# RamSaw/PipelineDP

Hardware: AMD Instinct MI355X
Metric: records/sec DPEngine.aggregate COUNT+SUM at 1/2/4/8 MI355X; % HBM roofline (higher is better)
Workload: dtype f64; 1 GPU; configs[1]: 1e+09 records / 1e+07 privacy ids / 1e+06 Zipf(1.1) partitions per GPU, COUNT+SUM+PRIVACY_ID_COUNT, private partition selection; records_per_gpu=1000000000, privacy_ids_per_gpu=10000000, partitions=1000000, max_partitions_contributed=8, max_contributions_per_partition=2, noise=laplace, selection=truncated_geometric, parallelism=pid-sharded x1, privacy_id_range_supplied=True

## Files before the change

### pipelinedp_amd/csrc/dpg_team.h

```cpp
#pragma once

#include "dpg_partition.h"

namespace dpg {

constexpr int kTeamIPT = 16;
#ifndef DPG_TEAM_PF
#define DPG_TEAM_PF 1
#endif
#ifndef DPG_TEAM_PF_PC
#define DPG_TEAM_PF_PC 1
#endif
#ifndef DPG_TEAM_WB
#define DPG_TEAM_WB 4
#endif
#ifndef DPG_TEAM_PAIR
#define DPG_TEAM_PAIR 1
#endif
#ifndef DPG_TEAM_DESC_AHEAD
#define DPG_TEAM_DESC_AHEAD 0
#endif
#ifndef DPG_TEAM_SCAN1
#define DPG_TEAM_SCAN1 1
#endif
constexpr uint32_t kTeamF = 2048;
constexpr int kTeamSub = kScatThreads * kTeamIPT;
constexpr uint64_t kTeamTimeout = 50000000ull;
constexpr uint32_t kTeamArriveStride = 32;

struct TeamSync {
    uint32_t *tot;
    uint32_t *arrive;
    uint32_t *abort;
    uint32_t *err;
    uint32_t *paths = nullptr;
};

template <class R>
constexpr size_t team_lds() {
    return sizeof(R) * (kTeamSub + 1) + (size_t)kTeamF * 12 + 4 * 4 + 64;
}

__device__ __forceinline__ uint32_t ld_agent(const uint32_t *p) {
    return __hip_atomic_load(p, __ATOMIC_RELAXED, __HIP_MEMORY_SCOPE_AGENT);
}

struct NoOp {
    __device__ __forceinline__ void operator()() const {}
};
template <class F = NoOp>
__device__ __forceinline__ bool team_barrier(const TeamSync &ts, uint32_t team, uint32_t target,
                                             uint32_t *sh_ok, const F &between = F{}) {
    asm volatile("s_waitcnt vmcnt(0)" ::: "memory");
    __syncthreads();
    uint32_t *ctr = ts.arrive + team * kTeamArriveStride;
    uint32_t seen = 0;
    if (threadIdx.x == 0) {
        __hip_atomic_fetch_add(ctr, 1u, __ATOMIC_RELAXED, __HIP_MEMORY_SCOPE_AGENT);
        seen = ld_agent(ctr);
    }
    between();
    if (threadIdx.x == 0) {
        const uint64_t t0 = wall_clock64();
        uint32_t ok = 1;
        for (; seen < target; seen = ld_agent(ctr)) {
            if (ld_agent(ts.abort)) {
                ok = 0;
                break;
            }
            if (wall_clock64() - t0 > kTeamTimeout) {
                atomicOr(ts.abort, 1u);
                atomicOr(ts.err, 8u);
                ok = 0;
                break;
            }
            __builtin_amdgcn_s_sleep(2);
        }
        *sh_ok = ok;
    }
    __syncthreads();
    return *sh_ok != 0;
}

struct PieceDesc {
    uint32_t n;
    uint32_t pad0;
    int64_t ostart;
    int64_t base0;
    uint32_t ppre[8];
    uint32_t dl[8];
    uint32_t cend[8];
    uint32_t pad1[2];
};
static_assert(sizeof(PieceDesc) == 128, "PieceDesc is two 64-byte scalar loads");

struct PieceTab {
    const int64_t *rbase;
    const uint32_t *cum;
    const uint32_t *tot;
    const uint32_t *ptot;
    const int64_t *ostart;
    uint32_t F1;
    const PieceDesc *desc = nullptr;
};

typedef uint32_t u32x16 __attribute__((ext_vector_type(16)));
__device__ __forceinline__ void sload_desc(const PieceDesc *p, u32x16 &a, u32x16 &b) {
    p = uniform_ptr(p);
    asm volatile("s_load_dwordx16 %0, %2, 0x0\n\ts_load_dwordx16 %1, %2, 0x40\n\ts_waitcnt lgkmcnt(0)"
                 : "=s"(a), "=s"(b)
                 : "s"(p)
                 : "memory");
}
__device__ __forceinline__ void sload_desc_early(const PieceDesc *p, u32x16 &a, u32x16 &b) {
    typedef const u32x16 __attribute__((address_space(4))) * ConstVec;
    const ConstVec q = (ConstVec)(uintptr_t)uniform_ptr(p);
    a = q[0];
    b = q[1];
}

struct PieceSpan {
    uint32_t bnd, dl0, ce0, dl1, ce1, pair;
};
__host__ __device__ inline PieceSpan team_resolve(const uint32_t (&ppre)[8], const uint32_t (&dl)[8],
                                                  const uint32_t (&ce)[8], uint32_t b0, uint32_t lim) {
    const uint32_t i0 = b0, i1 = b0 + (lim > 2u ? lim : 2u) - 2u;
    PieceSpan r{ppre[0], dl[0], ce[0], dl[0], ce[0], 0u};
    const uint32_t n0 = ~i0, n1 = ~i1;
    uint32_t m0[8], m1[8];
#pragma unroll
    for (int p = 1; p < 8; ++p) {
        m0[p] = (uint32_t)((int32_t)(ppre[p] + n0) >> 31);
        m1[p] = (uint32_t)((int32_t)(ppre[p] + n1) >> 31);
#ifdef __HIP_DEVICE_COMPILE__
        asm("" : "+s"(m0[p]), "+s"(m1[p]));
#endif
        r.dl0 ^= (r.dl0 ^ dl[p]) & m0[p];
        r.ce0 ^= (r.ce0 ^ ce[p]) & m0[p];
        r.dl1 ^= (r.dl1 ^ dl[p]) & m1[p];
        r.ce1 ^= (r.ce1 ^ ce[p]) & m1[p];
        r.bnd ^= (r.bnd ^ ppre[p]) & m1[p];
    }
    uint32_t mid = 0;
#pragma unroll
    for (int p = 1; p < 7; ++p)
        mid |= ~m0[p] & m1[p + 1] & (uint32_t)((int32_t)(ppre[p] - ppre[p + 1]) >> 31);
    r.pair = ~mid & 1u;
    return r;
}

__device__ __forceinline__ uint32_t team_addr_lookup(const u32x16 &da, const u32x16 &db, uint32_t b0,
                                                     uint32_t lim, uint32_t (&boff)[kTeamIPT / 2]) {
    uint32_t ppre[8], dl[8], ce[8];
#pragma unroll
    for (int p = 0; p < 8; ++p) {
        ppre[p] = da[6 + p];
        dl[p] = p < 2 ? da[14 + p] : db[p - 2];
        ce[p] = db[6 + p];
    }
    uint32_t vm = 0;
#pragma unroll
    for (int mm = 0; mm < kTeamIPT / 2; ++mm) {
        const uint32_t o = mm * 2 * kScatThreads + 2 * threadIdx.x;
        const uint32_t i = b0 + min(o, lim - 2);
        uint32_t d = dl[0], c = ce[0];
#pragma unroll
        for (int p = 1; p < 8; ++p) {
            const bool in = i >= ppre[p];
            d = in ? dl[p] : d;
            c = in ? ce[p] : c;
        }
        boff[mm] = (i + d) * 8u;
        vm |= (i < c ? 1u : 0u) << (2 * mm);
        vm |= (i + 1 < c ? 1u : 0u) << (2 * mm + 1);
    }
    return vm;
}
__device__ __forceinline__ uint32_t team_addr_pair(const PieceSpan &sp, uint32_t b0, uint32_t lim,
                                                   uint32_t (&boff)[kTeamIPT / 2]) {
    uint32_t vm = 0;
#pragma unroll
    for (int mm = 0; mm < kTeamIPT / 2; ++mm) {
        const uint32_t o = mm * 2 * kScatThreads + 2 * threadIdx.x;
        const uint32_t i = b0 + min(o, lim - 2);
        const bool in = i >= sp.bnd;
        const uint32_t d = in ? sp.dl1 : sp.dl0, c = in ? sp.ce1 : sp.ce0;
        boff[mm] = (i + d) * 8u;
        vm |= (i < c ? 1u : 0u) << (2 * mm);
        vm |= (i + 1 < c ? 1u : 0u) << (2 * mm + 1);
    }
    return vm;
}
template <class R>
__device__ __forceinline__ void team_fetch(const R *a, int64_t base0, uint32_t (&boff)[kTeamIPT / 2],
                                           uint32_t &vm, R (&rec)[kTeamIPT]) {
    static_assert(sizeof(R) == 8 && kTeamIPT == 16, "piece-mode teams read 8-byte records");
    asm volatile(""
                 : "+v"(boff[0]), "+v"(boff[1]), "+v"(boff[2]), "+v"(boff[3]), "+v"(boff[4]),
                   "+v"(boff[5]), "+v"(boff[6]), "+v"(boff[7]), "+v"(vm));
    const char *bp = reinterpret_cast<const char *>(a + base0);
#pragma unroll
    for (int mm = 0; mm < kTeamIPT / 2; ++mm) {
        R x0, x1;
        const u64x2 w = *reinterpret_cast<const u64x2 *>(bp + boff[mm]);
        const uint64_t w0 = w.x, w1 = w.y;
        __builtin_memcpy(&x0, &w0, sizeof(R));
        __builtin_memcpy(&x1, &w1, sizeof(R));
        rec[2 * mm] = x0;
        rec[2 * mm + 1] = x1;
    }
}

template <class R, bool kPc = false, bool kMulti = false>
__global__ __launch_bounds__(kScatThreads) void k_part2_team(SrcAoS<R> src,
                                                             const int64_t *seg_start,
                                                             const uint32_t *seg_cnt, uint32_t S,
                                                             uint32_t F2, R *out, int64_t *base_out,
                                                             uint32_t *tot_out, TeamSync ts,
                                                             PieceTab pt = PieceTab{},
                                                             uint32_t sub_cap = kTeamSub) {
    constexpr int IPT = kTeamIPT;
    constexpr int SUB = kTeamSub;
    constexpr uint32_t F = kTeamF;
    constexpr int DPT = F / kScatThreads;
    using W = Words<R>;
    extern __shared__ __attribute__((aligned(16))) char smem[];
    W *stage = reinterpret_cast<W *>(smem);
    uint32_t *cnt = reinterpret_cast<uint32_t *>(smem + sizeof(R) * (SUB + 1));
    uint32_t *dstart = cnt + F;
    uint32_t *cur = dstart + F + 1;
    uint32_t *sh16 = cur + F;
    __shared__ uint32_t sh_ok;
    const uint32_t team = blockIdx.x & 7u;
    const uint32_t T = gridDim.x >> 3;
    const uint32_t m = blockIdx.x >> 3;
    const int tid = threadIdx.x;
    const int lane = tid & 63, wv = tid >> 6;
    for (uint32_t d = tid; d < F; d += kScatThreads) cnt[d] = 0;
    __syncthreads();
    auto elem = [tid](int j) -> uint32_t {
        return (uint32_t)((j >> 1) * 2 * kScatThreads + 2 * tid + (j & 1));
    };
    auto share = [&](uint32_t s, int64_t &st, uint32_t &n, uint32_t &b0, uint32_t &lim) {
        n = __builtin_amdgcn_readfirstlane(kPc ? pt.ptot[s] : seg_cnt[s]);
        const int64_t st0 = kPc ? pt.ostart[s] : seg_start[s];
        st = (int64_t)(((uint64_t)__builtin_amdgcn_readfirstlane((uint32_t)((uint64_t)st0 >> 32)) << 32) |
                       (uint32_t)__builtin_amdgcn_readfirstlane((uint32_t)st0));
        const uint32_t q = kPc ? (((n + T - 1) / T + 1) & ~1u) : (n + T - 1) / T;
        b0 = min(n, m * q);
        lim = min(n, b0 + q) - b0;
    };
    R rec[IPT];
    uint32_t vmask = ~0u;
    auto load = [&](int64_t base, uint32_t lim) {
        if (lim >= 2) {
#pragma unroll
            for (int mm = 0; mm < IPT / 2; ++mm) {
                const uint32_t o = mm * 2 * kScatThreads + 2 * tid;
                const uint32_t a = min(o, lim - 2);
                R x0, x1;
                src.fetch2(base + a, x0, x1);
                rec[2 * mm] = a == o ? x0 : x1;
                rec[2 * mm + 1] = x1;
            }
        } else {
#pragma unroll
            for (int j = 0; j < IPT; ++j) rec[j] = lim ? src.fetch(base) : R{};
        }
    };
    auto load_pieces = [&](uint32_t s, uint32_t b0, uint32_t lim) {
        uint32_t ppre[8], dl[8], pc[8];
        const int64_t rb0 = pt.rbase[s];
        const int64_t base0 = (int64_t)(((uint64_t)__builtin_amdgcn_readfirstlane((uint32_t)((uint64_t)rb0 >> 32)) << 32) |
                                        (uint32_t)__builtin_amdgcn_readfirstlane((uint32_t)rb0));
        uint32_t acc = 0;
#pragma unroll
        for (int p = 0; p < 8; ++p) {
            const uint32_t off = __builtin_amdgcn_readfirstlane(
                (uint32_t)(pt.rbase[(size_t)p * pt.F1 + s] - rb0));
            pc[p] = __builtin_amdgcn_readfirstlane(pt.cum[(size_t)p * pt.F1 + s]);
            ppre[p] = acc;
            dl[p] = off - acc;
            acc += (pc[p] + 1u) & ~1u;
        }
        const char *bp = reinterpret_cast<const char *>(src.a + base0);
        uint32_t vm = 0;
#pragma unroll
        for (int mm = 0; mm < IPT / 2; ++mm) {
            const uint32_t o = mm * 2 * kScatThreads + 2 * tid;
            const uint32_t i = b0 + min(o, lim - 2);
            uint32_t d = dl[0], c = pc[0] + ppre[0];
#pragma unroll
            for (int p = 1; p < 8; ++p) {
                const bool in = i >= ppre[p];
                d = in ? dl[p] : d;
                c = in ? pc[p] + ppre[p] : c;
            }
            R x0, x1;
            const uint32_t boff = (i + d) * (uint32_t)sizeof(R);
            static_assert(sizeof(R) == 8, "piece-mode teams read 8-byte records");
            const u64x2 w = *reinterpret_cast<const u64x2 *>(bp + boff);
            const uint64_t w0 = w.x, w1 = w.y;
            __builtin_memcpy(&x0, &w0, sizeof(R));
            __builtin_memcpy(&x1, &w1, sizeof(R));
            rec[2 * mm] = x0;
            rec[2 * mm + 1] = x1;
            vm |= (i < c ? 1u : 0u) << (2 * mm);
            vm |= (i + 1 < c ? 1u : 0u) << (2 * mm + 1);
        }
        vmask = vm;
    };
    auto load_pieces_desc = [&](const u32x16 &da, const u32x16 &db, uint32_t b0, uint32_t lim) {
        uint32_t boff[IPT / 2];
        uint32_t vm = team_addr_lookup(da, db, b0, lim, boff);
        team_fetch<R>(src.a, (int64_t)(((uint64_t)da[5] << 32) | da[4]), boff, vm, rec);
        vmask = vm;
    };
    auto load_span = [&](const PieceSpan &sp, int64_t base0, const PieceDesc *dp, uint32_t b0,
                         uint32_t lim) {
        uint32_t boff[IPT / 2];
        uint32_t vm;
        if (sp.pair) {
            vm = team_addr_pair(sp, b0, lim, boff);
        } else {
            u32x16 da, db;
            sload_desc(dp, da, db);
            vm = team_addr_lookup(da, db, b0, lim, boff);
        }
        team_fetch<R>(src.a, base0, boff, vm, rec);
        vmask = vm;
    };
    uint32_t k = 0;
    constexpr bool kPF = DPG_TEAM_PF && (!kPc || DPG_TEAM_PF_PC) && !kMulti;
    auto share_q = [&](uint32_t n) -> uint32_t {
        return kPc ? (((n + T - 1) / T + 1) & ~1u) : (n + T - 1) / T;
    };
    auto next_nonempty = [&](uint32_t s) -> uint32_t {
        for (; s < S; s += 8) {
            const uint32_t n = __builtin_amdgcn_readfirstlane(kPc ? pt.ptot[s] : seg_cnt[s]);
            if (n != 0 && share_q(n) <= sub_cap) break;
        }
        return s;
    };
    int64_t pf_st = 0;
    uint32_t pf_n = 0, pf_b0 = 0, pf_lim = 0;
    constexpr bool use_desc = kPc && kPF;
    constexpr bool kPair = use_desc && DPG_TEAM_PAIR;
    constexpr bool kAhead = use_desc && DPG_TEAM_DESC_AHEAD;
    PieceSpan pf_sp{};
    int64_t pf_base0 = 0;
    u32x16 pf_da = {}, pf_db = {};
    uint32_t n_pair = 0, n_lookup = 0;
    auto take_desc = [&](const u32x16 &da, const u32x16 &db) {
        pf_n = __builtin_amdgcn_readfirstlane(da[0]);
        pf_st = (int64_t)(((uint64_t)da[3] << 32) | da[2]);
        const uint32_t q = ((pf_n + T - 1) / T + 1) & ~1u;
        pf_b0 = min(pf_n, m * q);
        pf_lim = min(pf_n, pf_b0 + q) - pf_b0;
        if constexpr (kPair) {
            uint32_t ppre[8], dl[8], ce[8];
#pragma unroll
            for (int p = 0; p < 8; ++p) {
                ppre[p] = da[6 + p];
                dl[p] = p < 2 ? da[14 + p] : db[p - 2];
                ce[p] = db[6 + p];
            }
            pf_base0 = (int64_t)(((uint64_t)da[5] << 32) | da[4]);
            pf_sp = team_resolve(ppre, dl, ce, pf_b0, pf_lim);
            asm volatile(""
                         : "+s"(pf_sp.bnd), "+s"(pf_sp.dl0), "+s"(pf_sp.ce0), "+s"(pf_sp.dl1),
                           "+s"(pf_sp.ce1), "+s"(pf_sp.pair), "+s"(pf_b0), "+s"(pf_lim), "+s"(pf_base0));
        } else {
            pf_da = da;
            pf_db = db;
        }
    };
    auto issue_share = [&](uint32_t s) {
        if constexpr (kPair) {
            if (s < S) {
                n_pair += pf_sp.pair;
                n_lookup += 1u - pf_sp.pair;
            }
            load_span(pf_sp, pf_base0, pt.desc + min(s, S - 1), pf_b0, max(pf_lim, 2u));
        } else {
            load_pieces_desc(pf_da, pf_db, pf_b0, max(pf_lim, 2u));
        }
    };
    auto load_share = [&](uint32_t s) {
        if constexpr (kPc) {
            if constexpr (use_desc) {
                u32x16 da, db;
                sload_desc(pt.desc + min(s, S - 1), da, db);
                take_desc(da, db);
                issue_share(s);
                return;
            }
        }
        share(s, pf_st, pf_n, pf_b0, pf_lim);
        if constexpr (kPc) {
            vmask = 0;
            if (pf_lim > 0) load_pieces(s, pf_b0, pf_lim);
        } else {
            load(pf_st + pf_b0, pf_lim);
        }
    };
    uint32_t pf_s = S;
    if constexpr (kPF) {
        pf_s = next_nonempty(team);
        if (use_desc || pf_s < S) load_share(pf_s);
    }
    auto write_out = [&](int64_t st, uint32_t nv) {
        constexpr int WB = DPG_TEAM_WB;
        for (uint32_t k0 = 0; k0 < nv; k0 += WB * kScatThreads) {
            W x[WB];
            uint32_t dd[WB], kc[WB];
#pragma unroll
            for (int u = 0; u < WB; ++u) {
                kc[u] = min(k0 + u * kScatThreads + tid, nv - 1);
                x[u] = stage[kc[u]];
                dd[u] = src.digit(from_words<R>(x[u]));
            }
            uint32_t c1[WB], c2[WB];
#pragma unroll
            for (int u = 0; u < WB; ++u) {
                c1[u] = cur[dd[u]];
                c2[u] = dstart[dd[u]];
            }
#pragma unroll
            for (int u = 0; u < WB; ++u)
                *reinterpret_cast<W *>(&out[st + c1[u] + (kc[u] - c2[u])]) = x[u];
        }
    };
    for (uint32_t s = team; s < S; s += 8) {
        int64_t st;
        uint32_t n, b0, lim;
        if constexpr (kPF) {
            if (s == pf_s) {
                st = pf_st;
                n = pf_n;
                b0 = pf_b0;
                lim = pf_lim;
            } else {
                share(s, st, n, b0, lim);
            }
        } else {
            share(s, st, n, b0, lim);
        }
        if constexpr (kMulti) {
            if (n == 0 || share_q(n) <= sub_cap) continue;
        } else {
            if (n == 0) {
                if (m == 0)
                    for (uint32_t d = tid; d < F2; d += kScatThreads) {
                        base_out[(size_t)s * F2 + d] = st;
                        tot_out[(size_t)s * F2 + d] = 0;
                    }
                continue;
            }
            if (share_q(n) > sub_cap) continue;
        }
        auto team_starts = [&](const uint32_t *tt) {
            const uint32_t d0 = DPT * tid;
            uint32_t c[DPT], x = 0;
#pragma unroll
            for (int u = 0; u < DPT; ++u) {
                c[u] = ld_agent(&tt[d0 + u]);
                x += c[u];
            }
            uint32_t wt;
            uint32_t e = wave_excl_scan(x, wt);
            if (lane == 63) sh16[wv] = wt;
            __syncthreads();
#if DPG_TEAM_SCAN1
            uint32_t all;
            e += block_prefix16(sh16, all);
#else
#pragma unroll
            for (int w = 0; w < kScatThreads / 64; ++w)
                if (w < wv) e += sh16[w];
#endif
            uint32_t *tz = ts.tot + ((size_t)team * 3 + (k + 1) % 3) * F;
#pragma unroll
            for (int u = 0; u < DPT; ++u) {
                cur[d0 + u] += e;
                if (m == 0) {
                    if (d0 + u < F2) {
                        base_out[(size_t)s * F2 + d0 + u] = st + e;
                        tot_out[(size_t)s * F2 + d0 + u] = c[u];
                    }
                    __hip_atomic_store(&tz[d0 + u], 0u, __ATOMIC_RELAXED, __HIP_MEMORY_SCOPE_AGENT);
                }
                e += c[u];
            }
        };
        if constexpr (kMulti) {
            const uint32_t q = share_q(n);
            {
                uint32_t *tt = ts.tot + ((size_t)team * 3 + k % 3) * F;
                const uint32_t J = (q + sub_cap - 1) / sub_cap;
                auto load_part = [&](uint32_t j, uint32_t &lj) {
                    const uint32_t bj = b0 + j * sub_cap;
                    lj = lim > j * sub_cap ? min(sub_cap, lim - j * sub_cap) : 0u;
                    if constexpr (kPc) {
                        if constexpr (use_desc) {
                            u32x16 da, db;
                            sload_desc(pt.desc + s, da, db);
                            load_pieces_desc(da, db, bj, max(lj, 2u));
                        } else {
                            vmask = 0;
                            if (lj > 0) load_pieces(s, bj, lj);
                        }
                    } else {
                        load(st + bj, lj);
                    }
                };
                auto ok_elem = [&](int jj, uint32_t lj) {
                    bool ok = elem(jj) < lj;
                    if constexpr (kPc) ok = ok && ((vmask >> jj) & 1u);
                    return ok;
                };
                for (uint32_t j = 0; j < J; ++j) {
                    uint32_t lj;
                    load_part(j, lj);
#pragma unroll
                    for (int jj = 0; jj < IPT; ++jj) {
                        const bool ok = ok_elem(jj, lj);
                        atomicAdd(&cnt[ok ? src.digit(rec[jj]) : 0u], ok ? 1u : 0u);
                    }
                }
                __syncthreads();
                {
                    const uint32_t d0 = DPT * tid;
#pragma unroll
                    for (int u = 0; u < DPT; ++u) {
                        cur[d0 + u] = atomicAdd(&tt[d0 + u], cnt[d0 + u]);
                        cnt[d0 + u] = 0;
                    }
                }
                ++k;
                if (!team_barrier(ts, team, T * k, &sh_ok)) return;
                team_starts(tt);
                for (uint32_t j = 0; j < J; ++j) {
                    __syncthreads();
                    uint32_t lj;
                    load_part(j, lj);
                    uint32_t drm[IPT];
#pragma unroll
                    for (int jj = 0; jj < IPT; ++jj) {
                        const bool ok = ok_elem(jj, lj);
                        const uint32_t dg = ok ? src.digit(rec[jj]) : 0u;
                        const uint32_t rk = atomicAdd(&cnt[dg], ok ? 1u : 0u);
                        drm[jj] = ok ? (dg | (rk << 12)) : ~0u;
                    }
                    __syncthreads();
                    const uint32_t d0 = DPT * tid;
                    uint32_t c[DPT], x = 0;
#pragma unroll
                    for (int u = 0; u < DPT; ++u) {
                        c[u] = cnt[d0 + u];
                        x += c[u];
                    }
                    uint32_t wt;
                    uint32_t e = wave_excl_scan(x, wt);
                    if (lane == 63) sh16[wv] = wt;
                    __syncthreads();
                    uint32_t nvj = 0;
#if DPG_TEAM_SCAN1
                    e += block_prefix16(sh16, nvj);
#else
#pragma unroll
                    for (int w = 0; w < kScatThreads / 64; ++w) {
                        if (w < wv) e += sh16[w];
                        nvj += sh16[w];
                    }
#endif
#pragma unroll
                    for (int u = 0; u < DPT; ++u) {
                        dstart[d0 + u] = e;
                        cnt[d0 + u] = 0;
                        e += c[u];
                    }
                    __syncthreads();
#pragma unroll
                    for (int jj = 0; jj < IPT; ++jj) {
                        const uint32_t pos = drm[jj] != ~0u ? dstart[drm[jj] & 0xFFFu] + (drm[jj] >> 12)
                                                            : (uint32_t)SUB;
                        stage[pos] = to_words(rec[jj]);
                    }
                    __syncthreads();
                    write_out(st, nvj);
                    __syncthreads();
#pragma unroll
                    for (int u = 0; u < DPT; ++u) cur[d0 + u] += c[u];
                }
                __syncthreads();
                continue;
            }
        } else {
        uint32_t *tt = ts.tot + ((size_t)team * 3 + k % 3) * F;
        if constexpr (!kPF) load_share(s);
        u32x16 nda = {}, ndb = {};
        if constexpr (kAhead) sload_desc_early(pt.desc + min(s + 8, S - 1), nda, ndb);
        uint32_t dr[IPT];
        uint32_t nv = 0;
        {
            uint32_t dg[IPT];
            bool okv[IPT];
#pragma unroll
            for (int j = 0; j < IPT; ++j) {
                okv[j] = elem(j) < lim;
                if constexpr (kPc) okv[j] = okv[j] && ((vmask >> j) & 1u);
                dg[j] = okv[j] ? src.digit(rec[j]) : 0u;
            }
            uint32_t rk[IPT];
#pragma unroll
            for (int j = 0; j < IPT; ++j) rk[j] = atomicAdd(&cnt[dg[j]], okv[j] ? 1u : 0u);
#pragma unroll
            for (int j = 0; j < IPT; ++j) dr[j] = okv[j] ? (dg[j] | (rk[j] << 12)) : ~0u;
        }
        __syncthreads();
        {
            const uint32_t d0 = DPT * tid;
            uint32_t c[DPT], x = 0;
#pragma unroll
            for (int u = 0; u < DPT; ++u) {
                c[u] = cnt[d0 + u];
                x += c[u];
            }
            uint32_t o[DPT];
#pragma unroll
            for (int u = 0; u < DPT; ++u) o[u] = atomicAdd(&tt[d0 + u], c[u]);
            if constexpr (kAhead) {
                uint32_t ns = s + 8;
                const uint32_t nn = __builtin_amdgcn_readfirstlane(nda[0]);
                if (ns < S && (nn == 0 || share_q(nn) > sub_cap)) {
                    ns = next_nonempty(ns + 8);
                    u32x16 da, db;
                    sload_desc(pt.desc + min(ns, S - 1), da, db);
                    take_desc(da, db);
                } else {
                    take_desc(nda, ndb);
                }
                pf_s = ns;
            }
            uint32_t wt;
            uint32_t e = wave_excl_scan(x, wt);
            if (lane == 63) sh16[wv] = wt;
            __syncthreads();
#if DPG_TEAM_SCAN1
            e += block_prefix16(sh16, nv);
#else
#pragma unroll
            for (int w = 0; w < kScatThreads / 64; ++w) {
                if (w < wv) e += sh16[w];
                nv += sh16[w];
            }
#endif
#pragma unroll
            for (int u = 0; u < DPT; ++u) {
                dstart[d0 + u] = e;
                if constexpr (!kPF) cur[d0 + u] = o[u];
                cnt[d0 + u] = 0;
                e += c[u];
            }
            if (tid == 0) dstart[F] = nv;
            if constexpr (kPF) {
                __syncthreads();
#pragma unroll
                for (int j = 0; j < IPT; ++j) {
                    const uint32_t pos = dr[j] != ~0u ? dstart[dr[j] & 0xFFFu] + (dr[j] >> 12) : (uint32_t)SUB;
                    stage[pos] = to_words(rec[j]);
                }
#pragma unroll
                for (int u = 0; u < DPT; ++u) cur[d0 + u] = o[u];
                if constexpr (!kAhead) pf_s = next_nonempty(s + 8);
            }
        }
        ++k;
        auto prefetch = [&]() {
            if constexpr (kAhead) {
                issue_share(pf_s);
            } else if constexpr (kPF) {
                if (use_desc || pf_s < S) load_share(pf_s);
            }
        };
        if (!team_barrier(ts, team, T * k, &sh_ok, prefetch)) return;
        {
            const uint32_t d0 = DPT * tid;
            uint32_t c[DPT], x = 0;
#pragma unroll
            for (int u = 0; u < DPT; ++u) {
                c[u] = ld_agent(&tt[d0 + u]);
                x += c[u];
            }
            uint32_t wt;
            uint32_t e = wave_excl_scan(x, wt);
            if (lane == 63) sh16[wv] = wt;
            __syncthreads();
#if DPG_TEAM_SCAN1
            uint32_t all;
            e += block_prefix16(sh16, all);
#else
#pragma unroll
            for (int w = 0; w < kScatThreads / 64; ++w)
                if (w < wv) e += sh16[w];
#endif
            uint32_t *tz = ts.tot + ((size_t)team * 3 + (k + 1) % 3) * F;
#pragma unroll
            for (int u = 0; u < DPT; ++u) {
                cur[d0 + u] += e;
                if (m == 0) {
                    if (d0 + u < F2) {
                        base_out[(size_t)s * F2 + d0 + u] = st + e;
                        tot_out[(size_t)s * F2 + d0 + u] = c[u];
                    }
                    __hip_atomic_store(&tz[d0 + u], 0u, __ATOMIC_RELAXED, __HIP_MEMORY_SCOPE_AGENT);
                }
                e += c[u];
            }
        }
        if constexpr (!kPF) {
#pragma unroll
            for (int j = 0; j < IPT; ++j) {
                const uint32_t pos = dr[j] != ~0u ? dstart[dr[j] & 0xFFFu] + (dr[j] >> 12) : (uint32_t)SUB;
                stage[pos] = to_words(rec[j]);
            }
        }
        __syncthreads();
        {
            constexpr int WB = DPG_TEAM_WB;
            for (uint32_t k0 = 0; k0 < nv; k0 += WB * kScatThreads) {
                W x[WB];
                uint32_t dd[WB], kc[WB];
#pragma unroll
                for (int u = 0; u < WB; ++u) {
                    kc[u] = min(k0 + u * kScatThreads + tid, nv - 1);
                    x[u] = stage[kc[u]];
                    dd[u] = src.digit(from_words<R>(x[u]));
                }
                uint32_t c1[WB], c2[WB];
#pragma unroll
                for (int u = 0; u < WB; ++u) {
                    c1[u] = cur[dd[u]];
                    c2[u] = dstart[dd[u]];
                }
#pragma unroll
                for (int u = 0; u < WB; ++u)
                    *reinterpret_cast<W *>(&out[st + c1[u] + (kc[u] - c2[u])]) = x[u];
            }
        }
        __syncthreads();
        }
    }
    if constexpr (kPair) {
        if (ts.paths && tid == 0) {
            atomicAdd(&ts.paths[0], n_pair);
            atomicAdd(&ts.paths[1], n_lookup);
        }
    }
}

}
```

Baseline: 58.42 billion records/s.

## Pack team digit reservations into 64-bit atomics and split prefetch resolve/issue

Each thread's two per-digit team counters are now reserved with one 64-bit atomic add and read back with one 64-bit load, halving the cross-block atomic traffic in the team scatter. The prefetch is split into an address-resolve step and a fetch-issue step, so the fetch can later be deferred behind an optional scanner-wave scan of the totals. That scanner-wave path stays off by default. The writeback loop is fully unrolled with a fixed trip count. The packed atomic assumes the paired counters stay 8-byte aligned and cannot carry between halves.

```diff
diff --git a/pipelinedp_amd/csrc/dpg_team.h b/pipelinedp_amd/csrc/dpg_team.h
--- a/pipelinedp_amd/csrc/dpg_team.h
+++ b/pipelinedp_amd/csrc/dpg_team.h
@@ -23,6 +23,13 @@
 #ifndef DPG_TEAM_SCAN1
 #define DPG_TEAM_SCAN1 1
 #endif
+#ifndef DPG_TEAM_SCANW
+#define DPG_TEAM_SCANW 0
+#endif
+#ifndef DPG_TEAM_RSV_PAIR
+#define DPG_TEAM_RSV_PAIR 1
+#endif
+static_assert(DPG_TEAM_SCANW == 0 || DPG_TEAM_SCANW == 4, "scanner waves: 4 (8 digits a thread) or none");
 constexpr uint32_t kTeamF = 2048;
 constexpr int kTeamSub = kScatThreads * kTeamIPT;
 constexpr uint64_t kTeamTimeout = 50000000ull;
@@ -44,9 +51,35 @@
 __device__ __forceinline__ uint32_t ld_agent(const uint32_t *p) {
     return __hip_atomic_load(p, __ATOMIC_RELAXED, __HIP_MEMORY_SCOPE_AGENT);
 }
+__device__ __forceinline__ uint64_t ld_agent2(const uint32_t *p) {
+    return __hip_atomic_load(reinterpret_cast<const uint64_t *>(p), __ATOMIC_RELAXED,
+                             __HIP_MEMORY_SCOPE_AGENT);
+}
+__device__ __forceinline__ void team_reserve2(uint32_t *tt2, const uint32_t (&c)[2], uint32_t (&o)[2]) {
+#if DPG_TEAM_RSV_PAIR
+    const uint64_t old = __hip_atomic_fetch_add(reinterpret_cast<uint64_t *>(tt2),
+                                                (uint64_t)c[0] | ((uint64_t)c[1] << 32),
+                                                __ATOMIC_RELAXED, __HIP_MEMORY_SCOPE_AGENT);
+    o[0] = (uint32_t)old;
+    o[1] = (uint32_t)(old >> 32);
+#else
+    o[0] = atomicAdd(&tt2[0], c[0]);
+    o[1] = atomicAdd(&tt2[1], c[1]);
+#endif
+}
+__device__ __forceinline__ void team_totals2(const uint32_t *tt2, uint32_t (&c)[2]) {
+#if DPG_TEAM_RSV_PAIR
+    const uint64_t w = ld_agent2(tt2);
+    c[0] = (uint32_t)w;
+    c[1] = (uint32_t)(w >> 32);
+#else
+    c[0] = ld_agent(&tt2[0]);
+    c[1] = ld_agent(&tt2[1]);
+#endif
+}
 
 struct NoOp {
-    __device__ __forceinline__ void operator()() const {}
+    __device__ __forceinline__ void operator()(uint32_t &) const {}
 };
 template <class F = NoOp>
 __device__ __forceinline__ bool team_barrier(const TeamSync &ts, uint32_t team, uint32_t target,
@@ -59,7 +92,7 @@
         __hip_atomic_fetch_add(ctr, 1u, __ATOMIC_RELAXED, __HIP_MEMORY_SCOPE_AGENT);
         seen = ld_agent(ctr);
     }
-    between();
+    between(seen);
     if (threadIdx.x == 0) {
         const uint64_t t0 = wall_clock64();
         uint32_t ok = 1;
@@ -223,6 +256,7 @@
     constexpr int SUB = kTeamSub;
     constexpr uint32_t F = kTeamF;
     constexpr int DPT = F / kScatThreads;
+    static_assert(DPT == 2, "a thread reserves and reads its digits as one pair");
     using W = Words<R>;
     extern __shared__ __attribute__((aligned(16))) char smem[];
     W *stage = reinterpret_cast<W *>(smem);
@@ -236,6 +270,14 @@
     const uint32_t m = blockIdx.x >> 3;
     const int tid = threadIdx.x;
     const int lane = tid & 63, wv = tid >> 6;
+    constexpr bool kScan = DPG_TEAM_SCANW > 0 && !kMulti;
+    const uint32_t wvu = __builtin_amdgcn_readfirstlane((uint32_t)wv);
+    auto is_scan_wave = [&]() __attribute__((always_inline)) -> bool {
+        if constexpr (!kScan) return false;
+        uint32_t w = wvu;
+        asm volatile("" : "+s"(w));
+        return w < (uint32_t)DPG_TEAM_SCANW;
+    };
     for (uint32_t d = tid; d < F; d += kScatThreads) cnt[d] = 0;
     __syncthreads();
     auto elem = [tid](int j) -> uint32_t {
@@ -316,20 +358,6 @@
         team_fetch<R>(src.a, (int64_t)(((uint64_t)da[5] << 32) | da[4]), boff, vm, rec);
         vmask = vm;
     };
-    auto load_span = [&](const PieceSpan &sp, int64_t base0, const PieceDesc *dp, uint32_t b0,
-                         uint32_t lim) {
-        uint32_t boff[IPT / 2];
-        uint32_t vm;
-        if (sp.pair) {
-            vm = team_addr_pair(sp, b0, lim, boff);
-        } else {
-            u32x16 da, db;
-            sload_desc(dp, da, db);
-            vm = team_addr_lookup(da, db, b0, lim, boff);
-        }
-        team_fetch<R>(src.a, base0, boff, vm, rec);
-        vmask = vm;
-    };
     uint32_t k = 0;
     constexpr bool kPF = DPG_TEAM_PF && (!kPc || DPG_TEAM_PF_PC) && !kMulti;
     auto share_q = [&](uint32_t n) -> uint32_t {
@@ -351,12 +379,13 @@
     int64_t pf_base0 = 0;
     u32x16 pf_da = {}, pf_db = {};
     uint32_t n_pair = 0, n_lookup = 0;
-    auto take_desc = [&](const u32x16 &da, const u32x16 &db) {
+    auto take_desc = [&](const u32x16 &da, const u32x16 &db) __attribute__((always_inline)) {
         pf_n = __builtin_amdgcn_readfirstlane(da[0]);
         pf_st = (int64_t)(((uint64_t)da[3] << 32) | da[2]);
         const uint32_t q = ((pf_n + T - 1) / T + 1) & ~1u;
         pf_b0 = min(pf_n, m * q);
         pf_lim = min(pf_n, pf_b0 + q) - pf_b0;
+        pf_base0 = (int64_t)(((uint64_t)da[5] << 32) | da[4]);
         if constexpr (kPair) {
             uint32_t ppre[8], dl[8], ce[8];
 #pragma unroll
@@ -365,7 +394,6 @@
                 dl[p] = p < 2 ? da[14 + p] : db[p - 2];
                 ce[p] = db[6 + p];
             }
-            pf_base0 = (int64_t)(((uint64_t)da[5] << 32) | da[4]);
             pf_sp = team_resolve(ppre, dl, ce, pf_b0, pf_lim);
             asm volatile(""
                          : "+s"(pf_sp.bnd), "+s"(pf_sp.dl0), "+s"(pf_sp.ce0), "+s"(pf_sp.dl1),
@@ -375,34 +403,53 @@
             pf_db = db;
         }
     };
-    auto issue_share = [&](uint32_t s) {
+    uint32_t pf_boff[IPT / 2] = {};
+    uint32_t pf_vm = 0;
+    auto addr_share = [&](uint32_t s) __attribute__((always_inline)) {
+        const uint32_t lim = max(pf_lim, 2u);
         if constexpr (kPair) {
             if (s < S) {
                 n_pair += pf_sp.pair;
                 n_lookup += 1u - pf_sp.pair;
             }
-            load_span(pf_sp, pf_base0, pt.desc + min(s, S - 1), pf_b0, max(pf_lim, 2u));
-        } else {
-            load_pieces_desc(pf_da, pf_db, pf_b0, max(pf_lim, 2u));
-        }
-    };
-    auto load_share = [&](uint32_t s) {
-        if constexpr (kPc) {
-            if constexpr (use_desc) {
+            if (pf_sp.pair) {
+                pf_vm = team_addr_pair(pf_sp, pf_b0, lim, pf_boff);
+            } else {
                 u32x16 da, db;
                 sload_desc(pt.desc + min(s, S - 1), da, db);
-                take_desc(da, db);
-                issue_share(s);
-                return;
-            }
-        }
-        share(s, pf_st, pf_n, pf_b0, pf_lim);
-        if constexpr (kPc) {
+                pf_vm = team_addr_lookup(da, db, pf_b0, lim, pf_boff);
+            }
+        } else {
+            pf_vm = team_addr_lookup(pf_da, pf_db, pf_b0, lim, pf_boff);
+        }
+    };
+    auto fetch_share = [&]() __attribute__((always_inline)) {
+        team_fetch<R>(src.a, pf_base0, pf_boff, pf_vm, rec);
+        vmask = pf_vm;
+    };
+    auto resolve_share = [&](uint32_t s) __attribute__((always_inline)) {
+        if constexpr (use_desc) {
+            u32x16 da, db;
+            sload_desc(pt.desc + min(s, S - 1), da, db);
+            take_desc(da, db);
+            addr_share(s);
+        } else {
+            share(s, pf_st, pf_n, pf_b0, pf_lim);
+        }
+    };
+    auto issue_share = [&](uint32_t s) __attribute__((always_inline)) {
+        if constexpr (use_desc) {
+            fetch_share();
+        } else if constexpr (kPc) {
             vmask = 0;
             if (pf_lim > 0) load_pieces(s, pf_b0, pf_lim);
         } else {
             load(pf_st + pf_b0, pf_lim);
         }
+    };
+    auto load_share = [&](uint32_t s) __attribute__((always_inline)) {
+        resolve_share(s);
+        issue_share(s);
     };
     uint32_t pf_s = S;
     if constexpr (kPF) {
@@ -461,12 +508,9 @@
         }
         auto team_starts = [&](const uint32_t *tt) {
             const uint32_t d0 = DPT * tid;
-            uint32_t c[DPT], x = 0;
-#pragma unroll
-            for (int u = 0; u < DPT; ++u) {
-                c[u] = ld_agent(&tt[d0 + u]);
-                x += c[u];
-            }
+            uint32_t c[DPT];
+            team_totals2(&tt[d0], c);
+            const uint32_t x = c[0] + c[1];
             uint32_t wt;
             uint32_t e = wave_excl_scan(x, wt);
             if (lane == 63) sh16[wv] = wt;
@@ -531,9 +575,12 @@
                 __syncthreads();
                 {
                     const uint32_t d0 = DPT * tid;
+                    const uint32_t c[DPT] = {cnt[d0], cnt[d0 + 1]};
+                    uint32_t o[DPT];
+                    team_reserve2(&tt[d0], c, o);
 #pragma unroll
                     for (int u = 0; u < DPT; ++u) {
-                        cur[d0 + u] = atomicAdd(&tt[d0 + u], cnt[d0 + u]);
+                        cur[d0 + u] = o[u];
                         cnt[d0 + u] = 0;
                     }
                 }
@@ -628,8 +675,7 @@
                 x += c[u];
             }
             uint32_t o[DPT];
-#pragma unroll
-            for (int u = 0; u < DPT; ++u) o[u] = atomicAdd(&tt[d0 + u], c[u]);
+            team_reserve2(&tt[d0], c, o);
             if constexpr (kAhead) {
                 uint32_t ns = s + 8;
                 const uint32_t nn = __builtin_amdgcn_readfirstlane(nda[0]);
@@ -677,22 +723,79 @@
             }
         }
         ++k;
-        auto prefetch = [&]() {
+        auto prefetch_issue = [&]() __attribute__((always_inline)) {
+            if constexpr (kPF) {
+                if (use_desc || pf_s < S) issue_share(pf_s);
+            }
+        };
+        constexpr bool kDefer = kScan && use_desc;
+        auto prefetch = [&](uint32_t &seen) __attribute__((always_inline)) {
             if constexpr (kAhead) {
-                issue_share(pf_s);
+                addr_share(pf_s);
             } else if constexpr (kPF) {
-                if (use_desc || pf_s < S) load_share(pf_s);
+                if (use_desc || pf_s < S) resolve_share(pf_s);
+            }
+            if constexpr (kScan) {
+                asm volatile("" : "+v"(seen));
+                if (!kDefer || !is_scan_wave()) prefetch_issue();
+            } else {
+                prefetch_issue();
             }
         };
         if (!team_barrier(ts, team, T * k, &sh_ok, prefetch)) return;
-        {
+        if constexpr (kScan) {
+            constexpr int SD = F / (64 * (kScan ? DPG_TEAM_SCANW : 4));
+            static_assert(SD == 8, "four 8-byte loads per scanner thread");
+            uint32_t tv = tid;
+            asm volatile("" : "+v"(tv));
+            const uint32_t d0 = SD * tv;
+            uint32_t c[SD] = {}, e = 0;
+            const bool scan_wave = is_scan_wave();
+            if (scan_wave) {
+                uint64_t w[SD / 2];
+#pragma unroll
+                for (int u = 0; u < SD / 2; ++u) w[u] = ld_agent2(&tt[d0 + 2 * u]);
+                if constexpr (kDefer) prefetch_issue();
+                uint32_t x = 0;
+#pragma unroll
+                for (int u = 0; u < SD / 2; ++u) {
+                    c[2 * u] = (uint32_t)w[u];
+                    c[2 * u + 1] = (uint32_t)(w[u] >> 32);
+                    x += c[2 * u] + c[2 * u + 1];
+                }
+                uint32_t wt;
+                e = wave_excl_scan(x, wt);
+                if (lane == 63) sh16[wv] = wt;
+            }
+            __syncthreads();
+            if (scan_wave) {
+#pragma unroll
+                for (int w = 0; w + 1 < DPG_TEAM_SCANW; ++w) {
+                    const uint32_t y = sh16[w];
+                    e += (uint32_t)w < wvu ? y : 0u;
+                }
+                uint32_t *tz = ts.tot + ((size_t)team * 3 + (k + 1) % 3) * F;
+                if (m == 0) {
+#pragma unroll
+                    for (int u = 0; u < SD / 2; ++u)
+                        __hip_atomic_store(reinterpret_cast<uint64_t *>(&tz[d0 + 2 * u]), (uint64_t)0,
+                                           __ATOMIC_RELAXED, __HIP_MEMORY_SCOPE_AGENT);
+                }
+#pragma unroll
+                for (int u = 0; u < SD; ++u) {
+                    cur[d0 + u] += e;
+                    if (m == 0 && d0 + u < F2) {
+                        base_out[(size_t)s * F2 + d0 + u] = st + e;
+                        tot_out[(size_t)s * F2 + d0 + u] = c[u];
+                    }
+                    e += c[u];
+                }
+            }
+        } else {
             const uint32_t d0 = DPT * tid;
-            uint32_t c[DPT], x = 0;
-#pragma unroll
-            for (int u = 0; u < DPT; ++u) {
-                c[u] = ld_agent(&tt[d0 + u]);
-                x += c[u];
-            }
+            uint32_t c[DPT];
+            team_totals2(&tt[d0], c);
+            const uint32_t x = c[0] + c[1];
             uint32_t wt;
             uint32_t e = wave_excl_scan(x, wt);
             if (lane == 63) sh16[wv] = wt;
@@ -729,12 +832,18 @@
         __syncthreads();
         {
             constexpr int WB = DPG_TEAM_WB;
-            for (uint32_t k0 = 0; k0 < nv; k0 += WB * kScatThreads) {
+            constexpr int kWbIter = (SUB + WB * kScatThreads - 1) / (WB * kScatThreads);
+            uint32_t tv = tid;
+            asm volatile("" : "+v"(tv));
+#pragma unroll
+            for (int b = 0; b < kWbIter; ++b) {
+                const uint32_t k0 = (uint32_t)b * WB * kScatThreads;
+                if (k0 >= nv) break;
                 W x[WB];
                 uint32_t dd[WB], kc[WB];
 #pragma unroll
                 for (int u = 0; u < WB; ++u) {
-                    kc[u] = min(k0 + u * kScatThreads + tid, nv - 1);
+                    kc[u] = min(k0 + u * kScatThreads + tv, nv - 1);
                     x[u] = stage[kc[u]];
                     dd[u] = src.digit(from_words<R>(x[u]));
                 }
```

Result: no change. 58.19 billion records/s (-0.4%).
